# johnmartinsson/differentiable-mel-spectrogram

Hardware: AMD Instinct MI355X
Metric: spectrogram frames/sec (fwd+bwd) (higher is better)
Workload: dtype f32

## Files before the change

differentiable-mel-spectrogram_amd/capi.py:

```python
from __future__ import annotations

import ctypes as C
import os

_PKG_DIR = os.path.dirname(os.path.abspath(__file__))
LIB_PATH = os.environ.get("DMEL_LIB") or os.path.join(_PKG_DIR, "libdmel_hip.so")

DMEL_OK = 0
DMEL_ERR_INVALID_ARGUMENT = 1
DMEL_ERR_UNSUPPORTED = 2
DMEL_ERR_HIP = 3
DMEL_ERR_NO_DEVICE = 4
DMEL_ERR_OUT_OF_MEMORY = 5
DMEL_ERR_LAMBD_TRACKING = 6
DMEL_ERR_MAILBOX_TIMEOUT = 7
DMEL_FLAG_MFMA_BF16X3 = 8
DMEL_FLAG_CHECK_NFFT = 16
DMEL_FLAG_X_INDIRECT = 32
DMEL_FLAG_LOG = 1
DMEL_FLAG_FULL_WINDOW = 2
DMEL_FLAG_OUT_BF16 = 4
DMEL_DTYPE_F32, DMEL_DTYPE_BF16 = 0, 1
MAX_NFFT = 16384
MIN_FAST_NFFT = 32

SYMBOLS = (
    "dmel_abi_version", "dmel_n_fft", "dmel_window_host", "dmel_mel_fbanks_host", "dmel_contraction_partition_host", "dmel_last_error",
    "dmel_device_count", "dmel_plan_create", "dmel_plan_destroy", "dmel_plan_set_filterbank",
    "dmel_forward", "dmel_backward", "dmel_backward_ex", "dmel_backward_fb", "dmel_backward_x", "dmel_spectrogram", "dmel_plan_get_info",
    "dmel_plan_set_profiling", "dmel_plan_get_profile", "dmel_spectrogram_ex",
    "dmel_comm_unique_id", "dmel_comm_create", "dmel_comm_destroy", "dmel_comm_allreduce_async", "dmel_comm_wait",
    "dmel_comm_allreduce", "dmel_scratch_bytes", "dmel_plan_set_filterbank_dev", "dmel_forward_scratch", "dmel_forward_dev", "dmel_forward_dev_fixed", "dmel_backward_fb_dev", "dmel_backward_scratch", "dmel_plan_get_config",
    "dmel_plan_lambd_status", "dmel_plan_set_tracking", "dmel_plan_lambd_reset",
# ... 6 lines not shown
    "dmel_forward_lengths", "dmel_forward_dev_lengths",
)
TORCH_LIB_PATH = os.path.join(_PKG_DIR, "libdmel_torch.so")


class DmelConfig(C.Structure):
    _fields_ = [("n_points", C.c_int32), ("hop_length", C.c_int32), ("n_mels", C.c_int32),
                ("sample_rate", C.c_int32), ("f_min", C.c_double), ("f_max", C.c_double),
                ("normalize_window", C.c_int32), ("max_batch", C.c_int32)]


class DmelPlanInfo(C.Structure):
    _fields_ = [("n_fft", C.c_int32), ("n_freqs", C.c_int32), ("n_time", C.c_int32),
                ("frames_per_tile", C.c_int32), ("grid_fwd", C.c_int32), ("fb_blocks", C.c_int32),
                ("fb_blocks_dense", C.c_int32), ("lds_bytes", C.c_int32), ("kernel_path", C.c_int32),
                ("contraction", C.c_int32), ("wl_steps", C.c_int32)]

    def as_dict(self):
        return {k: int(getattr(self, k)) for k, _ in self._fields_}


class DmelLambdStatus(C.Structure):
    _fields_ = [("known", C.c_int32), ("lambd_seen", C.c_float), ("n_fft_seen", C.c_int32), ("seq_issued", C.c_uint32),
                ("seq_seen", C.c_uint32), ("rate", C.c_float), ("guards", C.c_int32), ("error", C.c_int32),
                ("error_seq", C.c_uint32), ("error_lambd", C.c_float), ("next_n_fft", C.c_int32), ("next_guards", C.c_int32),
                ("calls", C.c_uint32)]


class DmelProfile(C.Structure):
    _fields_ = [("prep_ms", C.c_double), ("fwd_ms", C.c_double), ("bwd_ms", C.c_double),
                ("prep_launches", C.c_int32), ("fwd_launches", C.c_int32), ("bwd_launches", C.c_int32)]
# ... 594 lines not shown
```

differentiable-mel-spectrogram_amd/csrc/dmel_api.cpp:

```cpp
#include "../../include/dmel.h"
#include "dmel_kernels.h"

#include <algorithm>
#include <cmath>
#include <cstdio>
#include <cstdlib>
#include <cstring>
#include <functional>
#include <initializer_list>
#include <map>
#include <mutex>
#include <string>
#include <unordered_set>
#include <vector>

namespace {

thread_local std::string g_err;

dmel_status fail(dmel_status st, const std::string& msg)
{
    g_err = msg;
    return st;
}
// ... 40 lines not shown
    int ent_b_floats = 0;
    int4* tile_ranges = nullptr;
    float* fb_dense = nullptr;
    float2* tw_long = nullptr;
    float* fbT = nullptr;
    int2* band = nullptr;
    int2* rowband = nullptr;
    float4* rowpk = nullptr;
    bool long_rows = false;
    uint4* ent_h = nullptr;
    float* fb_nyq = nullptr;
    float4* wl_b4 = nullptr;
    int2* wl_lane = nullptr;
    int* wl_merge = nullptr;
    int wl_phases = 0, wl_total4 = 0;
    int wl_len4[dmel::kWlMaxPhases] = {};
    int wl_mg[dmel::kWlMaxPhases] = {};
    void release()
    {
        if (tw1p == tw1) tw1p = nullptr;
        if (tw2p == tw2) tw2p = nullptr;
        void* ptrs[] = {tw1, tw2, tw1p, tw2p, ent_b, ent_pre, tile_ranges, fb_dense, tw_long, fbT, band, rowband, rowpk, ent_h, fb_nyq, wl_b4, wl_lane, wl_merge};
        for (void* q : ptrs) (void)hipFree(q);
        *this = NfftTables();
    }
};

}

struct dmel_plan {
// ... 426 lines not shown
                        const int m = 4 * pc.quad + j;
                        lanes[(size_t)ph * 64 + 4 * b + j] = make_int2(8 * k0, (fin && m < M) ? m : -1);
                        merge[(size_t)ph * 64 + 4 * b + j] = (4 * p1 + j) | ((4 * p2 + j) << 8) | (f1 << 16) | (f2 << 17);
                        if (m >= M) continue;
                        for (int st = 0; st < 4 * n4; ++st) {
                            const int f = k0 + st;
                            const float v = (f < tb.F && f >= pc.lo && f < pc.lo + pc.w) ? fb[(size_t)f * M + m] : 0.f;
                            float4& e = b4[base + (size_t)(st / 4) * 64 + 4 * b + j];
                            (st % 4 == 0 ? e.x : st % 4 == 1 ? e.y : st % 4 == 2 ? e.z : e.w) = v;
                        }
                    }
                }
                tb.wl_mg[ph] = mg;
                tb.wl_total4 += n4;
            }
            DMEL_HIP(hipMalloc(&tb.wl_lane, lanes.size() * sizeof(int2)));
            DMEL_HIP(hipMemcpy(tb.wl_lane, lanes.data(), lanes.size() * sizeof(int2), hipMemcpyHostToDevice));
            DMEL_HIP(hipMalloc(&tb.wl_merge, merge.size() * sizeof(int)));
            DMEL_HIP(hipMemcpy(tb.wl_merge, merge.data(), merge.size() * sizeof(int), hipMemcpyHostToDevice));
            DMEL_HIP(hipMalloc(&tb.wl_b4, std::max<size_t>(b4.size(), 64) * sizeof(float4)));
            if (!b4.empty()) DMEL_HIP(hipMemcpy(tb.wl_b4, b4.data(), b4.size() * sizeof(float4), hipMemcpyHostToDevice));
        }
        {
            const int nbpre = dmel::forward_nbpre(N);
            std::vector<float> pre((size_t)waves * 2 * nbpre * 64, 0.f);
            for (int w = 0; w < waves; ++w)
                for (int loc = 0; loc < 2; ++loc) {
                    const int4 tr = ranges[(size_t)w * 2 + loc];
                    const int n = std::min(tr.y, nbpre);
                    tb.pre_groups[w * 2 + loc] = (n + 3) / 4;
// ... 237 lines not shown
        }
        const size_t m1 = prof_mark(pl, s);
        prof_span(pl, m0, m1, 0);
        dmel::BigParams bp{};
        bp.x = x_cell ? nullptr : x; bp.x_ind = x_cell; bp.out = out; bp.tangent = tangent; bp.psum = sc.psum; bp.win2 = pl->big_win;
        bp.tw = tw; bp.chirp = bt.chirp; bp.hbr = bt.hbr; bp.zws = pl->big_z; bp.fbT = tb->fbT; bp.band = tb->band;
        bp.B = batch; bp.L = pl->cfg.n_points; bp.T = pl->T; bp.hop = pl->cfg.hop_length; bp.M = pl->cfg.n_mels;
        bp.nchunks = pl->nchunks; bp.N = N; bp.F = tb->F; bp.mode = mode; bp.Mfft = bt.M; bp.logM = bt.logM;
        bp.inv_L = 1.0f / (float)pl->cfg.n_points; bp.eps = (float)eps; bp.flags = flags; bp.remove_dc = remove_dc; bp.lam = lam;
        bp.split = split ? 1 : 0; bp.wodd = wodd;
        DMEL_HIP(dmel::launch_big(bp, s));
        prof_span(pl, m1, prof_mark(pl, s), 1);
        pl->info.n_fft = N; pl->info.n_freqs = tb->F; pl->info.n_time = pl->T;
        pl->info.kernel_path = 3; pl->info.frames_per_tile = pair ? 2 : 1; pl->info.grid_fwd = grid;
        pl->info.fb_blocks = 0; pl->info.fb_blocks_dense = 0; pl->info.lds_bytes = dmel::big_uses_global(bt.M) ? 0 : bt.M * 8;
        pl->info.contraction = -1; pl->info.wl_steps = 0;
        return DMEL_OK;
    }

    const bool fast = N >= dmel::kMinFastNfft && N <= dmel::kMaxFastNfft;
    const bool kernel_mean = fast && pl->cfg.n_points <= 32768;
    const bool need_sums = remove_dc && !kernel_mean && !*sums_done;
    const bool need_window = !fast || !dmel::forward_window_in_lds(N);
    const size_t m0 = prof_mark(pl, s);
    if (need_sums || need_window) {
        dmel::PrepParams pp{};
        pp.x = x; pp.psum = sc.psum; pp.win2 = sc.win;
        if (flags & DMEL_FLAG_X_INDIRECT) { pp.x_ind = reinterpret_cast<const float* const*>(x); pp.x = nullptr; }
        pp.B = need_sums ? batch : 0; pp.L = pl->cfg.n_points; pp.nchunks = pl->nchunks; pp.chunk = pl->chunk;
        pp.N = need_window ? N : 0; pp.normalize = pl->cfg.normalize_window; pp.win_half = win_half; pp.center = center;
        pp.lam = lam; pp.lam.role = dmel::kLamQuiet;
// ... 14 lines not shown
    const size_t m1 = prof_mark(pl, s);
    if (need_sums || need_window) prof_span(pl, m0, m1, 0);

    pl->info.n_fft = N; pl->info.n_freqs = tb->F; pl->info.n_time = pl->T;
    const float inv_L = 1.0f / (float)pl->cfg.n_points;
    if (N < dmel::kMinFastNfft) {
        dmel::NaiveParams np{};
        np.x = x_cell ? nullptr : x; np.x_ind = x_cell; np.out = out; np.tangent = tangent; np.psum = sc.psum; np.win2 = sc.win; np.fb = tb->fb_dense;
        np.B = batch; np.L = pl->cfg.n_points; np.T = pl->T; np.hop = pl->cfg.hop_length; np.M = pl->cfg.n_mels;
        np.nchunks = pl->nchunks; np.N = N; np.F = tb->F; np.mode = mode;
        np.inv_L = inv_L; np.eps = (float)eps; np.flags = flags; np.remove_dc = remove_dc; np.lam = lam;
        DMEL_HIP(dmel::launch_naive(np, s));
        prof_span(pl, m1, prof_mark(pl, s), 1);
        pl->info.kernel_path = 1; pl->info.frames_per_tile = 1; pl->info.grid_fwd = batch * pl->T;
        pl->info.fb_blocks = 0; pl->info.fb_blocks_dense = 0; pl->info.lds_bytes = (2 * N + 2 * tb->F) * 4;
        pl->info.contraction = -1; pl->info.wl_steps = 0;
        return DMEL_OK;
    }
    dmel::FwdParams fp{};
    if (flags & DMEL_FLAG_X_INDIRECT) {
        fp.x_ind = reinterpret_cast<const float* const*>(x);
        x = nullptr;
        flags &= ~DMEL_FLAG_X_INDIRECT;
    }
    fp.x = x; fp.out = out; fp.tangent = tangent; fp.psum = (remove_dc && !kernel_mean) ? sc.psum : nullptr; fp.win2 = sc.win;
    fp.tw1 = dmel::mode_pairs(mode) ? tb->tw1p : tb->tw1; fp.tw2 = dmel::mode_pairs(mode) ? tb->tw2p : tb->tw2; fp.ent_b = tb->ent_b; fp.tile_ranges = tb->tile_ranges; fp.ent_b_floats = tb->ent_b_floats; fp.ent_pre = tb->ent_pre;
    for (int i = 0; i < 16; ++i) fp.pre_groups[i] = tb->pre_groups[i];
    fp.B = batch; fp.L = pl->cfg.n_points; fp.T = pl->T; fp.hop = pl->cfg.hop_length; fp.M = pl->cfg.n_mels;
    fp.nchunks = pl->nchunks; fp.groups = tb->groups; fp.xch_groups = tb->xch_groups;
    const bool hsplit = (flags & DMEL_FLAG_MFMA_BF16X3) && mode == dmel::kTrain && tb->ent_h != nullptr && !lengths;
    if (hsplit) mode = dmel::kTrainH;
    static const int wlc_env = std::getenv("DMEL_WLC") ? std::atoi(std::getenv("DMEL_WLC")) : -1;
    const bool wl_compact = tb->wl_total4 * 4 <= 320;
    if (mode == dmel::kTrain && tb->wl_b4 != nullptr && wlc_env != 0 && (wl_compact || wlc_env > 0)) {
        const int wide_fpt = dmel::forward_has_wlc_wide(N) ? dmel::forward_frames_per_tile(N, dmel::kTrainWW) : 0;
        const bool wide = wide_fpt > 0 && wlc_env == 2 && !lengths;
        mode = wide ? dmel::kTrainWW : dmel::kTrainW;
        fp.wl_b4 = tb->wl_b4; fp.wl_lane = tb->wl_lane; fp.wl_phases = tb->wl_phases; fp.wl_total4 = tb->wl_total4;
        for (int i = 0; i < dmel::kWlMaxPhases; ++i) { fp.wl_len4[i] = tb->wl_len4[i]; fp.wl_mg[i] = tb->wl_mg[i]; }
        fp.wl_merge = tb->wl_merge;
    }
    const int fpt = dmel::forward_frames_per_tile(N, mode);
    fp.tiles_per_clip = (pl->T + fpt - 1) / fpt;
    fp.inv_L = inv_L; fp.eps = (float)eps; fp.flags = flags; fp.lam = lam;
    fp.remove_dc = remove_dc; fp.normalize = pl->cfg.normalize_window; fp.win_half = win_half;
    fp.spec_out = spec_out;
    fp.ent_h = tb->ent_h; fp.fb_nyq = tb->fb_nyq;
    static const int force_tpw = std::getenv("DMEL_TILES_PER_WG") ? std::atoi(std::getenv("DMEL_TILES_PER_WG")) : 0;
    int tpw = dmel::forward_tiles_per_wg(N, mode, batch, fp.tiles_per_clip);
    if (force_tpw == 1 || (force_tpw == 2 && dmel::forward_two_tiles(N, mode))) tpw = force_tpw;
    if (hsplit || lengths || (ml && ml->edges)) tpw = 1;
    fp.wgs_per_clip = (fp.tiles_per_clip + tpw - 1) / tpw;
    long long grid = (long long)batch * fp.wgs_per_clip;
    if (ml) {
        fp.ch_out = ml->ch_out; fp.ch_grid = (int)grid; fp.ch_list = ml->list; fp.ch_roles = ml->roles;
        for (int c = 0; c < dmel::kMaxChannels; ++c) fp.ch_val[c] = ml->vals[c];
// ... 9 lines not shown
    } else if (ml && ml->edges) {
        dmel::FwdBandParams bp{};
        static_cast<dmel::FwdParams&>(bp) = fp;
        for (int c = 0; c <= dmel::kMaxChannels; ++c) bp.band_edges[c] = ml->edges[std::min(c, ml->channels)];
        DMEL_HIP(dmel::launch_forward_band(N, mode, tpw, bp, (int)grid, s));
    } else {
        DMEL_HIP(dmel::launch_forward(N, mode, tpw, fp, (int)grid, s));
    }
    prof_span(pl, m1, prof_mark(pl, s), 1);
    pl->info.kernel_path = 0; pl->info.frames_per_tile = fpt; pl->info.grid_fwd = (int)grid;
    pl->info.fb_blocks = tb->n_entries; pl->info.fb_blocks_dense = tb->n_dense;
    pl->info.lds_bytes = dmel::forward_lds_bytes(N, mode);
    const bool spec_only = mode == dmel::kSpec || mode == dmel::kSpecTrain;
    pl->info.contraction = spec_only ? -1 : (dmel::mode_wlc(mode) ? 1 : (mode == dmel::kTrainH ? 2 : 0));
    pl->info.wl_steps = dmel::mode_wlc(mode) ? 4 * fp.wl_total4 : 0;
    return DMEL_OK;
}

dmel_status mailbox_status(const dmel_plan* pl)
{
    const unsigned long long w = dmel::mailbox_peek_error(pl->mailbox);
    if (w == 0) return DMEL_OK;
    return fail(DMEL_ERR_MAILBOX_TIMEOUT, "mailbox all-reduce: rank " + std::to_string((unsigned)(w & 0xffffffffu)) + " never arrived at exchange " +
                std::to_string((unsigned)(w >> 32)) + ": the reduced gradient of that step was NaN on this rank (dmel_mailbox_error clears this)");
}

dmel_status check_device(const dmel_plan* pl)
{
    int dev = -1;
    if (hipGetDevice(&dev) != hipSuccess) { (void)hipGetLastError(); return fail(DMEL_ERR_NO_DEVICE, "no current HIP device"); }
// ... 1716 lines not shown
```

differentiable-mel-spectrogram_amd/csrc/dmel_fwd_body.inc:

```
#if DMEL_FWD_MULTI
#define FWD_BO bo
#define FWD_LAM lam_args
#define FWD_WIN2 win2
#define FWD_LEADER grid_leader
#if DMEL_FWD_BAND
#define FWD_KERNEL dmel_fwd_band_kernel
#else
#define FWD_KERNEL dmel_fwd_multi_kernel
#endif
#else
#define FWD_BO b
#define FWD_LAM p.lam
#define FWD_WIN2 p.win2
#define FWD_LEADER blockIdx.x == 0
#if DMEL_FWD_LEN
#define FWD_KERNEL dmel_fwd_len_kernel
#else
#define FWD_KERNEL dmel_fwd_kernel
#endif
#endif
#if DMEL_FWD_LEN
#define FWD_PARAMS FwdLenParams
#define FWD_LC Lc
#define FWD_INV_L inv_Lc
// ... 170 lines not shown
        int l = boff4 + n4; l = l < p.wl_total4 ? l : p.wl_total4; l -= 1;
        return l > 0 ? l : 0;
    };
    auto wl_ring_init = [&](int n4, int boff4) {
        if constexpr (DMEL_WL_UNCOND) n4 = wl_last(n4, boff4);
        if constexpr (WLC) static_for<0, WL_DEPTH>([&](auto dd) { constexpr int d = decltype(dd)::value; asm volatile("" : "=v"(wl_ring[d])); wl_bload(wl_ring[d], d, n4, boff4); });
    };
    auto wl_prefetch = [&]() {
        if constexpr (WLC && WL_EARLY >= 1) {
            wl_li[0] = p.wl_lane[lane];
            wl_li[1] = p.wl_lane[(p.wl_phases > 1 ? 64 : 0) + lane];
            if constexpr (WL_EARLY >= 2) wl_ring_init(p.wl_len4[0], 0);
        }
    };

    const int j = (WPF > 1) ? 0 : lane / G;
    const int lg = (WPF > 1) ? (wave % WPF) * 64 + lane : lane % G;
    const int qp = lg / C, r = lg % C;
    unsigned* fctr = reinterpret_cast<unsigned*>(red) + 36;
    unsigned fmeet = 0;
    static_assert(WPF == 1 || (WAVES / WPF <= 4 && 36 + 4 <= kRedBytes / 4), "one counter per frame of the workgroup");
    auto sync_frame = [&]() {
        if constexpr (WPF > 1) {
            fmeet += WPF;
            unsigned* c = fctr + wave / WPF;
            __builtin_amdgcn_fence(__ATOMIC_RELEASE, "workgroup");
            if (lane == 0) __hip_atomic_fetch_add(c, 1u, __ATOMIC_RELAXED, __HIP_MEMORY_SCOPE_WORKGROUP);
            for (;;) {
                const unsigned v = __hip_atomic_load(c, __ATOMIC_RELAXED, __HIP_MEMORY_SCOPE_WORKGROUP);
                if ((int)((unsigned)__builtin_amdgcn_readfirstlane((int)v) - fmeet) >= 0) break;
// ... 106 lines not shown
            return;
        }
#if DMEL_FWD_LEN
        if (!len_ok || tile0 * FPT >= Tc) {
            fill_rows(tile0 * FPT, (tile0 + TPW) * FPT, len_ok);
            return;
        }
#endif
        if constexpr (WPF > 1) {
            if (tid < 4) fctr[tid] = 0u;
            __syncthreads();
        }
        if constexpr (TRAINLIKE || MODE == kSpecTrain) {
            if (wave == 0) { const float h = 0.5f * lam_tangent_scale(ls); if (lane == 0) red[kRedTan] = h; }
        }
        if constexpr (TW2_LDS) { if (tid < R * C) tw2l[tid] = p.tw2[tid]; }
        if constexpr (TW1_LDS) {
            constexpr int n16 = (R - 1) * G / 2;
            for (int i = tid; i < n16; i += THREADS)
                reinterpret_cast<float4*>(smem_raw + g.TW1_OFF)[i] = reinterpret_cast<const float4*>(p.tw1 + G)[i];
        }
        if constexpr (SPLIT && !IS_SPEC) {
            constexpr int first = 2 * F, count = SS * 2 - first;
            static_assert(count >= 0, "slot stride covers PD[0 .. N/2]");
            if constexpr (count > 0) {
                constexpr int CP = 1 << (ilog2(count - 1 > 0 ? count - 1 : 1) + 1);
                static_assert(count <= CP, "slot padding fits the zeroing loop");
#ifdef DMEL_ABLATE
                if (!(p.flags & 0x100000u))
#endif
// ... 311 lines not shown
                    static_for<0, R>([&](auto qq) {
                        constexpr int q = decltype(qq)::value;
                        v2f v;
                        if constexpr (TW1_LDS && DMEL_TW1_CHUNK > 0) {
                            if constexpr (q % TW1C == 0 && q + TW1C < R) {
                                __builtin_amdgcn_sched_barrier(0);
                                tw1_fetch(IC<q + TW1C>{});
                                __builtin_amdgcn_sched_barrier(0);
                            }
                            v = z[bitrev(q, LB)];
                            if constexpr (q != 0) v = cmul(v, tw1r[q]);
                        } else v = twiddled(qq, z[bitrev(q, LB)]);
                        z[bitrev(q, LB)] = v;
                        slf[q * EXS + lg] = v.x;
                    });
                    sync_frame();
                    float ure[R];
                    static_for<0, R>([&](auto bb) {
                        constexpr int bi = decltype(bb)::value;
                        ure[bi] = slf[qp * EXS + r + C * bi];
                    });
                    sync_frame();
                    static_for<0, R>([&](auto qq) {
                        constexpr int q = decltype(qq)::value;
                        slf[q * EXS + lg] = z[bitrev(q, LB)].y;
                    });
                    sync_frame();
                    static_for<0, R>([&](auto bb) {
                        constexpr int bi = decltype(bb)::value;
                        u[bi] = v2f{ure[bi], slf[qp * EXS + r + C * bi]};
// ... 73 lines not shown
                            znx[p1] = plane[(p1 == 0) ? midx0 : midx - R * p1];
                        });
                        sync_frame();
                        static_for<0, R>([&](auto pp1) { constexpr int p1 = decltype(pp1)::value; plane[pidx + R * p1] = zr[p1].y; });
                        sync_frame();
                    }
                    v2f pdk[PLANE ? R / 2 + 1 : 1];
                    const int slot_b = slot * (SS * 8);
                    const int base_a = slot_b + (qp + (RR + PADC) * p2) * 8;
                    const int base_b = slot_b + ((R - qp) + R * (R - 1) + (RR + PADC) * p2m) * 8;
                    const int obase = dir_a ? base_a : base_b;
                    const int ostep = dir_a ? R * 8 : -R * 8;
                    const bool nyq = q0 && (2 * p2 == C);
                    const int addr0 = nyq ? slot_b + (N / 2 + (WLC ? 0 : PADC * (C / 2))) * 8 : obase;
                    const bool w0 = dir_a || !q0 || nyq;
                    static_for<0, R / 2 + 1>([&](auto pp1) {
                        constexpr int p1 = decltype(pp1)::value;
                        constexpr int s_a = (p1 == R / 2) ? R / 2 : (R - 1 - p1);
                        constexpr int s_b = (p1 == R / 2) ? R / 2 : ((R - p1) % R);
                        const float send_x = (s_a == s_b) ? zr[s_a].x : (q0 ? zr[s_b].x : zr[s_a].x);
                        const float send_y = (s_a == s_b) ? zr[s_a].y : (q0 ? zr[s_b].y : zr[s_a].y);
                        v2f zn;
                        if constexpr (PLANE) {
                            zn = v2f{znx[p1], plane[(p1 == 0) ? midx0 : midx - R * p1]};
                        } else {
                            const int pull = (p1 == 0) ? pull0 : pull1;
                            const int got_x = __builtin_amdgcn_ds_bpermute(pull, __builtin_bit_cast(int, send_x));
                            const int got_y = __builtin_amdgcn_ds_bpermute(pull, __builtin_bit_cast(int, send_y));
                            zn = v2f{__builtin_bit_cast(float, got_x), __builtin_bit_cast(float, got_y)};
                        }
// ... 119 lines not shown
            const int fr = (FPW == 2) ? (row & 1) : 0, typ = (FPW == 2) ? (row >> 1) : (row & 1);
            const int a_lane = (wave * FPW + fr) * (SS * 8) + typ * 4;
            const int tA = t0 + wave * FPW;
            int off4 = 0;
            float* const out_clip = p.out + (size_t)FWD_BO * p.M * p.T;
            unsigned short* const outh_clip = reinterpret_cast<unsigned short*>(p.out) + (size_t)FWD_BO * p.M * p.T;
            float* const tan_clip = p.tangent ? p.tangent + (size_t)FWD_BO * p.M * p.T : nullptr;
#ifndef DMEL_WL_STAGE
#define DMEL_WL_STAGE 1
#endif
            constexpr int NST = (FPW == 1) ? 4 : 2;
            const bool staged = DMEL_WL_STAGE && p.wl_phases <= NST && p.M <= SS && !out_bf16 && (p.T & 3) == 0 && p.tangent != nullptr && SLOTS % 4 == 0;
            float sv[NST][2 * FPW];
            int sm[NST];
            static_for<0, NST>([&](auto pp) { sm[decltype(pp)::value] = -1; });
            int2 li_pref = (WL_EARLY >= 1) ? wl_li[0] : p.wl_lane[lane];
            int mi_pref = (FPW == 1 && p.wl_mg[0] != 0) ? p.wl_merge[lane] : 0;
            for (int ph = 0; ph < p.wl_phases; ++ph) {
                const int n4 = p.wl_len4[ph];
                const int2 li = li_pref;
#if DMEL_FWD_BAND
                const bool row_mine = li.y >= e_lo && li.y < e_hi;
                const int n4r = (!DMEL_BAND_SKIP || __any(row_mine)) ? n4 : 0;
#else
                const int n4r = n4;
#endif
                const int mi = mi_pref;
                if (ph + 1 < p.wl_phases) {
                    li_pref = p.wl_lane[(ph + 1) * 64 + lane];
                    if constexpr (FPW == 1) mi_pref = (p.wl_mg[ph + 1] != 0) ? p.wl_merge[(ph + 1) * 64 + lane] : 0;
                }
                if ((WL_EARLY < 2 && ph == 0) || (!DMEL_WL_NEXT && ph > 0)) wl_ring_init(n4, off4);
                off4 += n4;
                int aaddr = a_lane + li.x;
                floatx4 acc0 = {0.f, 0.f, 0.f, 0.f}, acc1 = {0.f, 0.f, 0.f, 0.f};
                float a_cur[4];
                static_for<0, 4>([&](auto uu) { constexpr int u = decltype(uu)::value; a_cur[u] = *reinterpret_cast<const float*>(smem_raw + aaddr + 8 * u); });
                auto group = [&](auto dd) {
                    constexpr int d = decltype(dd)::value;
                    float a_nxt[4];
                    static_for<0, 4>([&](auto uu) { constexpr int u = decltype(uu)::value; a_nxt[u] = *reinterpret_cast<const float*>(smem_raw + aaddr + 32 * (d + 1) + 8 * u); });
                    const floatx4 bq = wl_ring[d];
#ifdef DMEL_ABLATE
                    if (p.flags & 0x800u) { acc0[0] += a_cur[0] + a_cur[1] + a_cur[2] + a_cur[3] + bq[0] + bq[1] + bq[2] + bq[3]; static_for<0, 4>([&](auto uu) { constexpr int u = decltype(uu)::value; a_cur[u] = a_nxt[u]; }); return; }
#endif
                    acc0 = __builtin_amdgcn_mfma_f32_4x4x1f32(a_cur[0], bq[0], acc0, 0, 0, 0);
                    acc1 = __builtin_amdgcn_mfma_f32_4x4x1f32(a_cur[1], bq[1], acc1, 0, 0, 0);
                    acc0 = __builtin_amdgcn_mfma_f32_4x4x1f32(a_cur[2], bq[2], acc0, 0, 0, 0);
                    acc1 = __builtin_amdgcn_mfma_f32_4x4x1f32(a_cur[3], bq[3], acc1, 0, 0, 0);
                    static_for<0, 4>([&](auto uu) { constexpr int u = decltype(uu)::value; a_cur[u] = a_nxt[u]; });
                };
                int s4 = 0;
                const int ring_n4 = DMEL_WL_UNCOND ? wl_last(n4, off4 - n4) : n4;
                for (; s4 + WL_DEPTH <= n4r; s4 += WL_DEPTH) {
                    static_for<0, WL_DEPTH>([&](auto dd) {
                        constexpr int d = decltype(dd)::value;
                        group(dd);
                        wl_bload(wl_ring[d], s4 + d + WL_DEPTH, ring_n4, off4 - n4);
                        if constexpr (DMEL_WL_UNCOND) {
                            __builtin_amdgcn_sched_group_barrier(0x100, 2, 0);
                            __builtin_amdgcn_sched_group_barrier(0x008, 4, 0);
                            __builtin_amdgcn_sched_group_barrier(0x020, 1, 0);
                        }
                    });
                    aaddr += WL_DEPTH * 32;
                }
                static_for<0, WL_DEPTH - 1>([&](auto dd) { if (s4 + decltype(dd)::value < n4r) group(dd); });
                if (DMEL_WL_NEXT && ph + 1 < p.wl_phases) wl_ring_init(p.wl_len4[ph + 1], off4);
                floatx4 tot = acc0 + acc1;
                if constexpr (FPW == 1) {
                    const int mg = p.wl_mg[ph];
                    if (mg != 0) {
                        float r0 = tot[0], r1 = tot[1];
                        {
                            const int pa = (mi & 63) << 2;
                            const float t0 = __int_as_float(__builtin_amdgcn_ds_bpermute(pa, __float_as_int(r0)));
                            const float t1 = __int_as_float(__builtin_amdgcn_ds_bpermute(pa, __float_as_int(r1)));
                            if (mi & 0x10000) { r0 += t0; r1 += t1; }
                        }
                        if (mg & 2) {
                            const int pb = ((mi >> 8) & 63) << 2;
                            const float t0 = __int_as_float(__builtin_amdgcn_ds_bpermute(pb, __float_as_int(r0)));
                            const float t1 = __int_as_float(__builtin_amdgcn_ds_bpermute(pb, __float_as_int(r1)));
// ... 362 lines not shown
```

differentiable-mel-spectrogram_amd/csrc/dmel_kernels.h:

```cpp
#pragma once
#include <hip/hip_runtime.h>
#include <stdint.h>

namespace dmel {

constexpr int kWave = 64;
constexpr int kThreads = 256;
constexpr int kMaxChunks = 64;
constexpr int kMaxFastNfft = 16384;
constexpr int kMaxNfft = 16384;
constexpr int kMinFastNfft = 32;

__device__ __forceinline__ unsigned short bf16_bits(float v) { return __builtin_bit_cast(unsigned short, (__bf16)v); }

enum Mode : int { kTrain = 0, kInfer = 1, kSpec = 2, kSpecTrain = 3,
                  kTrainH = 4,
                  kTrainW = 5,
                  kTrainWW = 6 };
constexpr bool mode_wlc(int mode) { return mode == kTrainW || mode == kTrainWW; }
#ifndef DMEL_WLC_4096
#define DMEL_WLC_4096 0
#endif
#ifndef DMEL_WLC_512
#define DMEL_WLC_512 0
// ... 156 lines not shown
template <int N, bool PAIR, bool WL> struct FftPlanSel3 : FftPlanSel<N, PAIR> {};
#ifndef DMEL_WL512_WAVES
#define DMEL_WL512_WAVES 8
#endif
template <> struct FftPlanSel3<512, false, true> { static constexpr int R = 16, C = 2, PASSES = 1, WAVES = DMEL_WL512_WAVES, NBPRE = 20, MINW = 4, PAIRING = 1, SPLIT = 1; };

constexpr unsigned kFwdEdgeFirst = 0x40u;
int forward_resident_workgroups(int n_fft, int mode);
constexpr int kWinLdsMaxNfft = 4096;
constexpr int kRedBytes = 160;
constexpr int kRedTan = 32;
struct FftGeom {
    int N, R, C, G, FPW, PASSES, WAVES, NLOC, THREADS, SLOTS, MT, EX_STRIDE, SLOT_STRIDE_F2, NBPRE, MINW, LDS_BYTES, AUX_OFF, RED_OFF, WIN_LDS;
    int PAIRING, SPLIT, WIN_SYM, WPF, PLANE_PAD;
    int TW1_OFF;
};

constexpr int ex_stride(int G, int C) { return G + (G >= 32 ? C : 1); }
constexpr int z_index_host(int k, int R, int C) { return C == 1 ? k : k + (k / (R * R)) * 4; }
constexpr int slot_stride_f2(int N, int R, int C, int pairing = 0, int split = 0, bool wl = false)
{
    const int G = N / R;
    const int a = R * ex_stride(G, C) * (split ? 4 : 8);
    const int b = (z_index_host(pairing ? N / 2 : N - 1, R, C) + 1) * 8;
    const int need = a > b ? a : b;
    if (wl) return ((need + 127) / 128 * 128 + 64) / 8;
    return ((need + 127) / 128 * 128 + 48) / 8;
}

template <int N, bool PAIR = false, bool WL = false, bool WIDE = false> constexpr FftGeom geom()
{
// ... 14 lines not shown
    g.WIN_SYM = (g.WIN_LDS && P::SPLIT) ? 1 : 0;
    const int win = g.WIN_LDS ? (g.WIN_SYM ? (N / 2 + 1) * 8 : N * 8) : 0;
    g.AUX_OFF = g.SLOTS * g.SLOT_STRIDE_F2 * 8;
    g.RED_OFF = g.AUX_OFF + (xch > win ? xch : win);
    g.TW1_OFF = 0;
    if (WL) {
        const int tw1 = (P::R - 1) * g.G * 8;
        const int win16 = (win + 15) / 16 * 16;
        const int with_tw1 = g.AUX_OFF + win16 + tw1 + kRedBytes + ((P::C > 1 && N <= 2048) ? P::R * P::C * 8 : 0);
        const int per_cu_now = 163840 / (g.RED_OFF + kRedBytes + ((P::C > 1 && N <= 2048) ? P::R * P::C * 8 : 0));
#ifndef DMEL_WL_TW1LDS
#define DMEL_WL_TW1LDS 1
#endif
        if (DMEL_WL_TW1LDS && 163840 / with_tw1 >= per_cu_now) { g.TW1_OFF = g.AUX_OFF + win16; g.RED_OFF = g.TW1_OFF + tw1; }
        else g.RED_OFF = g.AUX_OFF + win16;
    }
    g.LDS_BYTES = g.RED_OFF + kRedBytes + ((P::C > 1 && N <= 2048) ? P::R * P::C * 8 : 0);
    return g;
}

template <int N, int MODE> constexpr FftGeom geom_mode() { return geom<N, mode_pairs(MODE), mode_wlc(MODE), MODE == kTrainWW>(); }
constexpr bool wlc_wide_size(int n_fft) { return false; }

struct FwdParams {
    const float* x;
    const float* const* x_ind;
    float* out;
    float* tangent;
    const float* psum;
    const float2* win2;
    const float2* tw1;
    const float2* tw2;
    const float* ent_b;
    const int4* tile_ranges;
    int ent_b_floats;
    const float* ent_pre;
    int pre_groups[16];
    int B, L, T, hop, M, nchunks, groups, tiles_per_clip;
    float inv_L, eps;
    LamArgs lam;
    unsigned flags;
    int remove_dc, normalize;
    int win_half;
    int wgs_per_clip;
    unsigned xch_groups;
    const uint4* ent_h;
    const float* fb_nyq;
    float* spec_out;
    const float4* wl_b4;
    const int2* wl_lane;
    int wl_phases, wl_total4;
    int wl_len4[kWlMaxPhases];
    const int* wl_merge;
    int wl_mg[kWlMaxPhases];
    int ch_out, ch_grid;
    unsigned ch_list, ch_roles;
    float ch_val[kMaxChannels];
};

struct FwdLenParams : FwdParams {
    const int* lengths;
};

struct FwdBandParams : FwdParams {
    int band_edges[kMaxChannels + 1];
};
// ... 11 lines not shown
hipError_t launch_prep(const PrepParams& p, hipStream_t s);
hipError_t launch_forward(int n_fft, int mode, int tiles_per_wg, const FwdParams& p, int grid, hipStream_t s);
hipError_t launch_forward_len(int n_fft, int mode, int tiles_per_wg, const FwdLenParams& p, int grid, hipStream_t s);
hipError_t forward_len_prepare_attributes();
hipError_t launch_forward_band(int n_fft, int mode, int tiles_per_wg, const FwdBandParams& p, int grid, hipStream_t s);
hipError_t forward_band_prepare_attributes();
int forward_tiles_per_wg(int n_fft, int mode, int batch, int tiles_per_clip);
bool forward_two_tiles(int n_fft, int mode);
int forward_lds_bytes(int n_fft, int mode);
int forward_frames_per_tile(int n_fft, int mode);
int forward_waves(int n_fft);
int forward_nbpre(int n_fft);
bool forward_plan_rc(int n_fft, bool pair, int* R, int* C);
bool forward_has_hsplit(int n_fft);
bool forward_has_wlc(int n_fft);
bool forward_wlc_one_frame(int n_fft);
bool forward_has_wlc_wide(int n_fft);
bool forward_window_in_lds(int n_fft);
hipError_t forward_prepare_attributes();

__device__ __forceinline__ const float* resolve_x(const float* x, const float* const* x_ind)
{
#if defined(__HIPCC__)
    if (x_ind) { typedef const float* cfp; return *(const __attribute__((address_space(4))) cfp*)x_ind; }
#endif
    return x;
}

struct NaiveParams {
    const float* const* x_ind;
// ... 156 lines not shown
```

include/dmel.h:

```cpp
#ifndef DMEL_H
#define DMEL_H

#include <stddef.h>
#include <stdint.h>

#ifdef __cplusplus
extern "C" {
#endif

#define DMEL_ABI_VERSION 5

typedef enum dmel_status {
    DMEL_OK = 0,
    DMEL_ERR_INVALID_ARGUMENT = 1,
    DMEL_ERR_UNSUPPORTED = 2,
    DMEL_ERR_HIP = 3,
    DMEL_ERR_NO_DEVICE = 4,
    DMEL_ERR_OUT_OF_MEMORY = 5,
    DMEL_ERR_LAMBD_TRACKING = 6,
    DMEL_ERR_MAILBOX_TIMEOUT = 7
} dmel_status;

typedef struct dmel_config {
    int32_t n_points;
// ... 2 lines not shown
    int32_t sample_rate;
    double f_min;
    double f_max;
    int32_t normalize_window;
    int32_t max_batch;
} dmel_config;

typedef struct dmel_plan dmel_plan;

#define DMEL_FLAG_LOG 1u
#define DMEL_FLAG_FULL_WINDOW 2u
#define DMEL_FLAG_OUT_BF16 4u
#define DMEL_FLAG_MFMA_BF16X3 8u
#define DMEL_FLAG_CHECK_NFFT 16u
#define DMEL_FLAG_X_INDIRECT 32u
#define DMEL_DTYPE_F32 0
#define DMEL_DTYPE_BF16 1


int32_t dmel_abi_version(void);

int32_t dmel_n_fft(float lambd);

dmel_status dmel_window_host(float lambd, int32_t n_fft, int32_t normalize, float* window, float* dwindow);

dmel_status dmel_mel_fbanks_host(int32_t n_freqs, double f_min, double f_max, int32_t n_mels,
                                 int32_t sample_rate, float* fb);

dmel_status dmel_contraction_partition_host(const int32_t* units, int32_t n_tiles, int32_t waves, int32_t* own, int32_t* n_pieces,
                                            int32_t* piece_wave, int32_t* piece_tile, int32_t* piece_first, int32_t* piece_units);
// ... 142 lines not shown
dmel_status dmel_backward_band(dmel_plan* plan, const void* grad_out, int32_t grad_dtype, const float* tangent, int32_t batch, int32_t channels,
                               const int32_t* band_edges, int32_t accumulate, float* dlambd, void* scratch, void* stream);

typedef struct dmel_plan_info {
    int32_t n_fft;
    int32_t n_freqs;
    int32_t n_time;
    int32_t frames_per_tile;
    int32_t grid_fwd;
    int32_t fb_blocks;
    int32_t fb_blocks_dense;
    int32_t lds_bytes;
    int32_t kernel_path;
    int32_t contraction;
    int32_t wl_steps;
} dmel_plan_info;
dmel_status dmel_plan_get_info(const dmel_plan* plan, dmel_plan_info* info);

typedef struct dmel_profile {
    double prep_ms;
    double fwd_ms;
    double bwd_ms;
    int32_t prep_launches, fwd_launches, bwd_launches;
} dmel_profile;
dmel_status dmel_plan_set_profiling(dmel_plan* plan, int32_t enable);
dmel_status dmel_plan_get_profile(dmel_plan* plan, dmel_profile* profile);

#ifdef __cplusplus
}
#endif
// ... 2 lines not shown
```

Before: 211.0 million.

## Keep tail of mel filterbank B operands resident in dead LDS for n_fft 1024

```diff
diff --git a/differentiable-mel-spectrogram_amd/capi.py b/differentiable-mel-spectrogram_amd/capi.py
--- a/differentiable-mel-spectrogram_amd/capi.py
+++ b/differentiable-mel-spectrogram_amd/capi.py
@@ -17,6 +17,7 @@
 DMEL_FLAG_MFMA_BF16X3 = 8
 DMEL_FLAG_CHECK_NFFT = 16
 DMEL_FLAG_X_INDIRECT = 32
+DMEL_FLAG_WL_RING = 128
 DMEL_FLAG_LOG = 1
 DMEL_FLAG_FULL_WINDOW = 2
 DMEL_FLAG_OUT_BF16 = 4
@@ -53,7 +54,7 @@
     _fields_ = [("n_fft", C.c_int32), ("n_freqs", C.c_int32), ("n_time", C.c_int32),
                 ("frames_per_tile", C.c_int32), ("grid_fwd", C.c_int32), ("fb_blocks", C.c_int32),
                 ("fb_blocks_dense", C.c_int32), ("lds_bytes", C.c_int32), ("kernel_path", C.c_int32),
-                ("contraction", C.c_int32), ("wl_steps", C.c_int32)]
+                ("contraction", C.c_int32), ("wl_steps", C.c_int32), ("wl_resident_steps", C.c_int32)]
 
     def as_dict(self):
         return {k: int(getattr(self, k)) for k, _ in self._fields_}
diff --git a/differentiable-mel-spectrogram_amd/csrc/dmel_api.cpp b/differentiable-mel-spectrogram_amd/csrc/dmel_api.cpp
--- a/differentiable-mel-spectrogram_amd/csrc/dmel_api.cpp
+++ b/differentiable-mel-spectrogram_amd/csrc/dmel_api.cpp
@@ -78,6 +78,7 @@
     int2* wl_lane = nullptr;
     int* wl_merge = nullptr;
     int wl_phases = 0, wl_total4 = 0;
+    int wl_res4 = 0;
     int wl_len4[dmel::kWlMaxPhases] = {};
     int wl_mg[dmel::kWlMaxPhases] = {};
     void release()
@@ -534,6 +535,11 @@
                 tb.wl_mg[ph] = mg;
                 tb.wl_total4 += n4;
             }
+            {
+                const int cap = dmel::forward_wlb_groups(N);
+                const int res = std::min(tb.wl_total4, cap);
+                tb.wl_res4 = (res > 0 && tb.wl_total4 - res <= dmel::kWlRegGroups) ? res : 0;
+            }
             DMEL_HIP(hipMalloc(&tb.wl_lane, lanes.size() * sizeof(int2)));
             DMEL_HIP(hipMemcpy(tb.wl_lane, lanes.data(), lanes.size() * sizeof(int2), hipMemcpyHostToDevice));
             DMEL_HIP(hipMalloc(&tb.wl_merge, merge.size() * sizeof(int)));
@@ -801,7 +807,7 @@
         pl->info.n_fft = N; pl->info.n_freqs = tb->F; pl->info.n_time = pl->T;
         pl->info.kernel_path = 3; pl->info.frames_per_tile = pair ? 2 : 1; pl->info.grid_fwd = grid;
         pl->info.fb_blocks = 0; pl->info.fb_blocks_dense = 0; pl->info.lds_bytes = dmel::big_uses_global(bt.M) ? 0 : bt.M * 8;
-        pl->info.contraction = -1; pl->info.wl_steps = 0;
+        pl->info.contraction = -1; pl->info.wl_steps = 0; pl->info.wl_resident_steps = 0;
         return DMEL_OK;
     }
 
@@ -846,7 +852,7 @@
         prof_span(pl, m1, prof_mark(pl, s), 1);
         pl->info.kernel_path = 1; pl->info.frames_per_tile = 1; pl->info.grid_fwd = batch * pl->T;
         pl->info.fb_blocks = 0; pl->info.fb_blocks_dense = 0; pl->info.lds_bytes = (2 * N + 2 * tb->F) * 4;
-        pl->info.contraction = -1; pl->info.wl_steps = 0;
+        pl->info.contraction = -1; pl->info.wl_steps = 0; pl->info.wl_resident_steps = 0;
         return DMEL_OK;
     }
     dmel::FwdParams fp{};
@@ -871,7 +877,9 @@
         fp.wl_b4 = tb->wl_b4; fp.wl_lane = tb->wl_lane; fp.wl_phases = tb->wl_phases; fp.wl_total4 = tb->wl_total4;
         for (int i = 0; i < dmel::kWlMaxPhases; ++i) { fp.wl_len4[i] = tb->wl_len4[i]; fp.wl_mg[i] = tb->wl_mg[i]; }
         fp.wl_merge = tb->wl_merge;
-    }
+        if (!wide && !lengths && !ml && !(flags & (DMEL_FLAG_WL_RING | DMEL_FLAG_OUT_BF16))) fp.wl_res4 = tb->wl_res4;
+    }
+    flags &= ~DMEL_FLAG_WL_RING;
     const int fpt = dmel::forward_frames_per_tile(N, mode);
     fp.tiles_per_clip = (pl->T + fpt - 1) / fpt;
     fp.inv_L = inv_L; fp.eps = (float)eps; fp.flags = flags; fp.lam = lam;
@@ -911,6 +919,7 @@
     const bool spec_only = mode == dmel::kSpec || mode == dmel::kSpecTrain;
     pl->info.contraction = spec_only ? -1 : (dmel::mode_wlc(mode) ? 1 : (mode == dmel::kTrainH ? 2 : 0));
     pl->info.wl_steps = dmel::mode_wlc(mode) ? 4 * fp.wl_total4 : 0;
+    pl->info.wl_resident_steps = 4 * fp.wl_res4;
     return DMEL_OK;
 }
 
diff --git a/differentiable-mel-spectrogram_amd/csrc/dmel_fwd_body.inc b/differentiable-mel-spectrogram_amd/csrc/dmel_fwd_body.inc
--- a/differentiable-mel-spectrogram_amd/csrc/dmel_fwd_body.inc
+++ b/differentiable-mel-spectrogram_amd/csrc/dmel_fwd_body.inc
@@ -208,6 +208,64 @@
         }
     };
 
+#if !DMEL_FWD_MULTI && !DMEL_FWD_LEN
+    constexpr bool WLB = WLC && g.WLB_BYTES > 0 && TPW == 1;
+#else
+    constexpr bool WLB = false;
+#endif
+    static_assert(!WLB || (WPF == 1 && PASSES == 1 && WL_DEPTH >= kWlRegGroups && 38 <= kRedBytes / 4), "resident B operands: one-wave frames, the ring's registers hold the rest");
+    constexpr int WLB_TURNS = WLB ? (g.WLB_BYTES / kWlbGroupBytes + WAVES - 1) / WAVES : 1;
+#ifndef DMEL_WLB_T
+#define DMEL_WLB_T 0
+#endif
+    const int wres = (WLB && !(DMEL_WLB_T & 1)) ? p.wl_res4 : 0;
+    const int wreg = p.wl_total4 - wres;
+    floatx4 wlb_stage[WLB_TURNS];
+    unsigned* wlb_ctr = reinterpret_cast<unsigned*>(red) + 36;
+    auto wlb_lane = [&]() -> int {
+        int l = (int)__builtin_amdgcn_mbcnt_hi(~0u, __builtin_amdgcn_mbcnt_lo(~0u, 0u));
+        if constexpr ((DMEL_WLB_T & 16) != 0) asm volatile("" : "+v"(l));
+        return l;
+    };
+    auto wlb_signal = [&](int which) {
+        __builtin_amdgcn_fence(__ATOMIC_RELEASE, "workgroup");
+        if (wlb_lane() == 0) __hip_atomic_fetch_add(wlb_ctr + which, 1u, __ATOMIC_RELAXED, __HIP_MEMORY_SCOPE_WORKGROUP);
+    };
+    auto wlb_wait = [&](int which) {
+        for (;;) {
+            const unsigned v = __hip_atomic_load(wlb_ctr + which, __ATOMIC_RELAXED, __HIP_MEMORY_SCOPE_WORKGROUP);
+            if (__builtin_amdgcn_readfirstlane((int)v) >= WAVES) break;
+            __builtin_amdgcn_s_sleep(1);
+        }
+        __builtin_amdgcn_fence(__ATOMIC_ACQUIRE, "workgroup");
+    };
+    auto wlb_request = [&]() {
+        if constexpr (WLB) {
+#ifndef DMEL_WLB_BOUND
+            if (wres > 0) static_for<0, WLB_TURNS>([&](auto ii) {
+                constexpr int i = decltype(ii)::value;
+                const int piece = (i * WAVES + wave) * 64 + wlb_lane();
+                wlb_stage[i] = __builtin_bit_cast(floatx4, __builtin_amdgcn_raw_buffer_load_b128(rbw, (piece < wres * 64 ? piece : 0) * 16, __builtin_amdgcn_readfirstlane(wreg) * kWlbGroupBytes, 0));
+            });
+#endif
+        }
+    };
+    auto wlb_land = [&]() {
+        if constexpr (WLB) {
+#ifndef DMEL_WLB_BOUND
+            if (wres > 0) {
+                wlb_wait(0);
+                static_for<0, WLB_TURNS>([&](auto ii) {
+                    constexpr int i = decltype(ii)::value;
+                    const int piece = (i * WAVES + wave) * 64 + wlb_lane();
+                    if (piece < wres * 64) *reinterpret_cast<floatx4*>(smem_raw + g.WLB_OFF + piece * 16) = wlb_stage[i];
+                });
+                wlb_signal(1);
+            }
+#endif
+        }
+    };
+
     const int j = (WPF > 1) ? 0 : lane / G;
     const int lg = (WPF > 1) ? (wave % WPF) * 64 + lane : lane % G;
     const int qp = lg / C, r = lg % C;
@@ -344,6 +402,7 @@
         if constexpr (TRAINLIKE || MODE == kSpecTrain) {
             if (wave == 0) { const float h = 0.5f * lam_tangent_scale(ls); if (lane == 0) red[kRedTan] = h; }
         }
+        if constexpr (WLB) { if (tid < 2) wlb_ctr[tid] = 0u; }
         if constexpr (TW2_LDS) { if (tid < R * C) tw2l[tid] = p.tw2[tid]; }
         if constexpr (TW1_LDS) {
             constexpr int n16 = (R - 1) * G / 2;
@@ -685,6 +744,9 @@
                         z[bitrev(q, LB)] = v;
                         slf[q * EXS + lg] = v.x;
                     });
+#ifndef DMEL_WLB_BOUND
+                    if constexpr (WLB) { if (wres > 0) wlb_signal(0); }
+#endif
                     sync_frame();
                     float ure[R];
                     static_for<0, R>([&](auto bb) {
@@ -788,6 +850,7 @@
                     const bool nyq = q0 && (2 * p2 == C);
                     const int addr0 = nyq ? slot_b + (N / 2 + (WLC ? 0 : PADC * (C / 2))) * 8 : obase;
                     const bool w0 = dir_a || !q0 || nyq;
+                    if constexpr (WLB && pass == PASSES - 1) { wlb_request(); __builtin_amdgcn_sched_barrier(0); }
                     static_for<0, R / 2 + 1>([&](auto pp1) {
                         constexpr int p1 = decltype(pp1)::value;
                         constexpr int s_a = (p1 == R / 2) ? R / 2 : (R - 1 - p1);
@@ -937,6 +1000,8 @@
             float sv[NST][2 * FPW];
             int sm[NST];
             static_for<0, NST>([&](auto pp) { sm[decltype(pp)::value] = -1; });
+            const bool wlb_on = WLB && wres > 0;
+            bool wlb_ready = false;
             int2 li_pref = (WL_EARLY >= 1) ? wl_li[0] : p.wl_lane[lane];
             int mi_pref = (FPW == 1 && p.wl_mg[0] != 0) ? p.wl_merge[lane] : 0;
             for (int ph = 0; ph < p.wl_phases; ++ph) {
@@ -953,17 +1018,20 @@
                     li_pref = p.wl_lane[(ph + 1) * 64 + lane];
                     if constexpr (FPW == 1) mi_pref = (p.wl_mg[ph + 1] != 0) ? p.wl_merge[(ph + 1) * 64 + lane] : 0;
                 }
-                if ((WL_EARLY < 2 && ph == 0) || (!DMEL_WL_NEXT && ph > 0)) wl_ring_init(n4, off4);
+                const int first4 = off4;
+                int nring = n4r, ninit = n4;
+                if constexpr (WLB) { if (wlb_on) { nring = wreg - first4; nring = nring < n4r ? nring : n4r; nring = nring > 0 ? nring : 0; ninit = nring; } }
+                if (((WL_EARLY < 2 && ph == 0) || (!DMEL_WL_NEXT && ph > 0)) && ninit > (wlb_on ? 0 : -1)) wl_ring_init(ninit, off4);
+                if constexpr (WLB) { if (ph == 0) wlb_land(); }
                 off4 += n4;
                 int aaddr = a_lane + li.x;
                 floatx4 acc0 = {0.f, 0.f, 0.f, 0.f}, acc1 = {0.f, 0.f, 0.f, 0.f};
                 float a_cur[4];
                 static_for<0, 4>([&](auto uu) { constexpr int u = decltype(uu)::value; a_cur[u] = *reinterpret_cast<const float*>(smem_raw + aaddr + 8 * u); });
-                auto group = [&](auto dd) {
+                auto group_b = [&](auto dd, const floatx4 bq) {
                     constexpr int d = decltype(dd)::value;
                     float a_nxt[4];
                     static_for<0, 4>([&](auto uu) { constexpr int u = decltype(uu)::value; a_nxt[u] = *reinterpret_cast<const float*>(smem_raw + aaddr + 32 * (d + 1) + 8 * u); });
-                    const floatx4 bq = wl_ring[d];
 #ifdef DMEL_ABLATE
                     if (p.flags & 0x800u) { acc0[0] += a_cur[0] + a_cur[1] + a_cur[2] + a_cur[3] + bq[0] + bq[1] + bq[2] + bq[3]; static_for<0, 4>([&](auto uu) { constexpr int u = decltype(uu)::value; a_cur[u] = a_nxt[u]; }); return; }
 #endif
@@ -973,13 +1041,14 @@
                     acc1 = __builtin_amdgcn_mfma_f32_4x4x1f32(a_cur[3], bq[3], acc1, 0, 0, 0);
                     static_for<0, 4>([&](auto uu) { constexpr int u = decltype(uu)::value; a_cur[u] = a_nxt[u]; });
                 };
+                auto group = [&](auto dd) { group_b(dd, wl_ring[decltype(dd)::value]); };
                 int s4 = 0;
-                const int ring_n4 = DMEL_WL_UNCOND ? wl_last(n4, off4 - n4) : n4;
-                for (; s4 + WL_DEPTH <= n4r; s4 += WL_DEPTH) {
+                const int ring_n4 = DMEL_WL_UNCOND ? wl_last(ninit, first4) : ninit;
+                for (; s4 + WL_DEPTH <= nring; s4 += WL_DEPTH) {
                     static_for<0, WL_DEPTH>([&](auto dd) {
                         constexpr int d = decltype(dd)::value;
                         group(dd);
-                        wl_bload(wl_ring[d], s4 + d + WL_DEPTH, ring_n4, off4 - n4);
+                        wl_bload(wl_ring[d], s4 + d + WL_DEPTH, ring_n4, first4);
                         if constexpr (DMEL_WL_UNCOND) {
                             __builtin_amdgcn_sched_group_barrier(0x100, 2, 0);
                             __builtin_amdgcn_sched_group_barrier(0x008, 4, 0);
@@ -988,8 +1057,31 @@
                     });
                     aaddr += WL_DEPTH * 32;
                 }
-                static_for<0, WL_DEPTH - 1>([&](auto dd) { if (s4 + decltype(dd)::value < n4r) group(dd); });
-                if (DMEL_WL_NEXT && ph + 1 < p.wl_phases) wl_ring_init(p.wl_len4[ph + 1], off4);
+                static_for<0, WL_DEPTH - 1>([&](auto dd) { if (s4 + decltype(dd)::value < nring) group(dd); });
+                if constexpr (WLB) {
+                    if (wlb_on && nring < n4r) {
+                        aaddr += (nring - s4) * 32;
+#ifndef DMEL_WLB_BOUND
+                        if (!wlb_ready) { wlb_wait(1); wlb_ready = true; }
+#endif
+                        int baddr = g.WLB_OFF + lane * 16 + (first4 + nring - wreg) * kWlbGroupBytes;
+                        auto ldsb = [&](int byte) -> floatx4 { return *reinterpret_cast<const floatx4*>(smem_raw + byte); };
+                        floatx4 b_cur = ldsb(baddr);
+                        for (int gq = nring; gq < n4r; ++gq) {
+                            floatx4 b_nxt = b_cur;
+                            if constexpr (!(DMEL_WLB_T & 4)) { if (gq + 1 < n4r) b_nxt = ldsb(baddr + kWlbGroupBytes); }
+                            group_b(IC<0>{}, b_cur);
+                            if constexpr ((DMEL_WLB_T & 4) != 0) { if (gq + 1 < n4r) b_nxt = ldsb(baddr + kWlbGroupBytes); }
+                            b_cur = b_nxt;
+                            aaddr += 32; baddr += kWlbGroupBytes;
+                        }
+                    }
+                }
+                if (DMEL_WL_NEXT && ph + 1 < p.wl_phases) {
+                    int nnext = p.wl_len4[ph + 1];
+                    if constexpr (WLB) { if (wlb_on) { const int h = wreg - off4; nnext = h < nnext ? h : nnext; } }
+                    if (nnext > (wlb_on ? 0 : -1)) wl_ring_init(nnext, off4);
+                }
                 floatx4 tot = acc0 + acc1;
                 if constexpr (FPW == 1) {
                     const int mg = p.wl_mg[ph];
diff --git a/differentiable-mel-spectrogram_amd/csrc/dmel_kernels.h b/differentiable-mel-spectrogram_amd/csrc/dmel_kernels.h
--- a/differentiable-mel-spectrogram_amd/csrc/dmel_kernels.h
+++ b/differentiable-mel-spectrogram_amd/csrc/dmel_kernels.h
@@ -194,7 +194,10 @@
     int N, R, C, G, FPW, PASSES, WAVES, NLOC, THREADS, SLOTS, MT, EX_STRIDE, SLOT_STRIDE_F2, NBPRE, MINW, LDS_BYTES, AUX_OFF, RED_OFF, WIN_LDS;
     int PAIRING, SPLIT, WIN_SYM, WPF, PLANE_PAD;
     int TW1_OFF;
-};
+    int WLB_OFF, WLB_BYTES;
+};
+constexpr int kWlRegGroups = 6;
+constexpr int kWlbGroupBytes = 1024;
 
 constexpr int ex_stride(int G, int C) { return G + (G >= 32 ? C : 1); }
 constexpr int z_index_host(int k, int R, int C) { return C == 1 ? k : k + (k / (R * R)) * 4; }
@@ -239,12 +242,23 @@
 #endif
         if (DMEL_WL_TW1LDS && 163840 / with_tw1 >= per_cu_now) { g.TW1_OFF = g.AUX_OFF + win16; g.RED_OFF = g.TW1_OFF + tw1; }
         else g.RED_OFF = g.AUX_OFF + win16;
+#ifndef DMEL_WLB_LDS
+#define DMEL_WLB_LDS 1
+#endif
+        if (DMEL_WLB_LDS && N == 1024 && !WIDE && g.TW1_OFF != 0) {
+            const int dead = g.RED_OFF - g.AUX_OFF;
+            g.WLB_OFF = g.AUX_OFF;
+            g.WLB_BYTES = (dead + kWlbGroupBytes - 1) / kWlbGroupBytes * kWlbGroupBytes;
+            g.RED_OFF = g.WLB_OFF + g.WLB_BYTES;
+        }
     }
     g.LDS_BYTES = g.RED_OFF + kRedBytes + ((P::C > 1 && N <= 2048) ? P::R * P::C * 8 : 0);
     return g;
 }
 
 template <int N, int MODE> constexpr FftGeom geom_mode() { return geom<N, mode_pairs(MODE), mode_wlc(MODE), MODE == kTrainWW>(); }
+static_assert(geom<1024, false, true>().WLB_BYTES == 12 * kWlbGroupBytes && geom<1024, false, true>().WLB_OFF % 16 == 0, "n_fft 1024: twelve resident groups of B operands");
+static_assert(2 * geom<1024, false, true>().LDS_BYTES <= 163840, "n_fft 1024, kTrainW: two workgroups per CU");
 constexpr bool wlc_wide_size(int n_fft) { return false; }
 
 struct FwdParams {
@@ -275,6 +289,7 @@
     const float4* wl_b4;
     const int2* wl_lane;
     int wl_phases, wl_total4;
+    int wl_res4;
     int wl_len4[kWlMaxPhases];
     const int* wl_merge;
     int wl_mg[kWlMaxPhases];
@@ -316,6 +331,7 @@
 bool forward_plan_rc(int n_fft, bool pair, int* R, int* C);
 bool forward_has_hsplit(int n_fft);
 bool forward_has_wlc(int n_fft);
+inline int forward_wlb_groups(int n_fft) { return n_fft == 1024 && wlc_size(1024) ? geom<1024, false, true>().WLB_BYTES / kWlbGroupBytes : 0; }
 bool forward_wlc_one_frame(int n_fft);
 bool forward_has_wlc_wide(int n_fft);
 bool forward_window_in_lds(int n_fft);
diff --git a/include/dmel.h b/include/dmel.h
--- a/include/dmel.h
+++ b/include/dmel.h
@@ -40,6 +40,7 @@
 #define DMEL_FLAG_MFMA_BF16X3 8u
 #define DMEL_FLAG_CHECK_NFFT 16u
 #define DMEL_FLAG_X_INDIRECT 32u
+#define DMEL_FLAG_WL_RING 128u
 #define DMEL_DTYPE_F32 0
 #define DMEL_DTYPE_BF16 1
 
@@ -212,6 +213,7 @@
     int32_t kernel_path;
     int32_t contraction;
     int32_t wl_steps;
+    int32_t wl_resident_steps;
 } dmel_plan_info;
 dmel_status dmel_plan_get_info(const dmel_plan* plan, dmel_plan_info* info);
 
```

After: 204.6 million. 0.969x the previous value.
